# TiagoMSSantos/MobileRayTracer

Hardware: AMD Instinct MI355X
Metric: Mrays/s + ms/frame, Conference OBJ 1920×1080 4spp, 1/2/4/8 GPU (higher is better)
Workload: dtype f32; 1 GPU; conference_1920x1080_4spp_pathtracer_depth5; rendered_pixels=2058240, spp=4, max_depth=5, samples_light=1, parallelism=single GPU

## Files before the change

### include/mobilert_amd.h

```cpp
#ifndef MOBILERT_AMD_H
#define MOBILERT_AMD_H

#include <stddef.h>
#include <stdint.h>

#ifdef __cplusplus
extern "C" {
#endif

typedef struct mrt_renderer mrt_renderer;

typedef struct mrt_config {
    int32_t width;
    int32_t height;
    int32_t threads;
    int32_t shader;
    int32_t sceneIndex;
    int32_t samplesPixel;
    int32_t samplesLight;
    int32_t repeats;
    int32_t accelerator;
    int32_t printStdOut;
    const char *objFilePath;
    const char *mtlFilePath;
// ... 138 lines not shown
int mrt_set_pixel_sampler(mrt_renderer *r, int32_t kind, float value);
int mrt_set_max_point(mrt_renderer *r, const float *maxPoint);
typedef struct mrt_view {
    int32_t kind;
    float position[3], lookAt[3], up[3];
    float a, b;
} mrt_view;
int mrt_render_views(mrt_renderer *r, const mrt_view *views, int32_t nViews, int32_t *bitmaps);
int mrt_render_views_device(mrt_renderer *r, const mrt_view *views, int32_t nViews,
                            int32_t *d_bitmaps, int32_t *d_packed, void *stream);
int mrt_set_tuning(mrt_renderer *r, int32_t key, int32_t value);
int mrt_get_tuning(const mrt_renderer *r, int32_t key, int32_t *value);
int mrt_primary_hits(mrt_renderer *r, int32_t *kind, int32_t *index, float *t);
int64_t mrt_triangle_bvh(const mrt_config *cfg, float *boxes, int32_t *offsets, int32_t *counts, int32_t *order);
int64_t mrt_walk_tree(const mrt_config *cfg, uint32_t *nodes, float *grid, int32_t *root);
int mrt_walk_stack(const mrt_config *cfg, int32_t *out);
int64_t mrt_plan_spill(int64_t threads, int32_t stackNeed, int64_t availBytes);
int64_t mrt_regular_grid(const mrt_config *cfg, int32_t kind, float *world, int32_t *start, int32_t *items);
int mrt_grid_box_test(int32_t kind, const float *prim, const float *box);
int64_t mrt_decode_texture(const char *path, int32_t *dims, uint8_t *texels);
int mrt_plan_queues(const mrt_queue_plan_request *request, mrt_queue_plan *plan);

int mrt_sample_tables(float *shader, float *sampler, float *trig);

int mrt_kat_slab(const float *boxes, const float *orig, const float *dir, int32_t n, int32_t *out);
int mrt_kat_triangle(const float *tris, const float *orig, const float *dir, int32_t n, int32_t *hit, float *t);
int mrt_kat_accumulate(const float *rgb, int32_t nSlots, int32_t spp, int32_t sampleBase, int32_t width,
                       int32_t height, int32_t mode, int32_t *bitmap, int32_t *launched);
int mrt_trace_rays(mrt_renderer *r, const float *orig, const float *dir, const float *dist, const int32_t *src,
                   int32_t n, int32_t any, int32_t *kind, int32_t *index, float *t);
// ... 142 lines not shown
```

### mobileraytracer_amd/__init__.py

```python
import contextlib
import ctypes
import dataclasses
import threading
import time
from typing import List, Optional

import numpy as np

from . import _native

SHADER_WHITTED = 1
SHADER_PATH_TRACER = 2
ACC_BVH = 3
RAY_DEPTH_MAX = 6


@dataclasses.dataclass
class Config:
    width: int = 256
    height: int = 256
    threads: int = 1
    shader: int = SHADER_WHITTED
    sceneIndex: int = 0
    samplesPixel: int = 1
# ... 662 lines not shown


def walk_tree(config: Config):
    lib = _native.lib()
    c = config.to_c()
    n = lib.mrt_walk_tree(ctypes.byref(c), None, None, None)
    if n < 0:
        raise RuntimeError(lib.mrt_last_error().decode())
    grid = np.empty(6, np.float32)
    root = np.empty(3, np.int32)
    lib.mrt_walk_tree(ctypes.byref(c), None, _ptr(grid), _ptr(root))
    nodes = np.empty((n, 4 * int(root[2])), np.uint32)
    if lib.mrt_walk_tree(ctypes.byref(c), _ptr(nodes), _ptr(grid), _ptr(root)) != n:
        raise RuntimeError(lib.mrt_last_error().decode())
    return nodes, grid, root


def walk_stack(config: Config) -> dict:
    out = np.zeros(6, np.int32)
    c = config.to_c()
    _native.check(_native.lib().mrt_walk_stack(ctypes.byref(c), _ptr(out)))
    return {"need": int(out[0]), "quantized": bool(out[1]), "refDepth": int(out[2]), "walkDepth": int(out[3]),
            "wideDepth": int(out[4]), "spillDepth": int(out[5])}


def plan_spill(threads: int, stack_need: int, avail_bytes: int = 0) -> int:
    n = _native.lib().mrt_plan_spill(int(threads), int(stack_need), int(avail_bytes))
    if n < 0:
        raise RuntimeError(_native.lib().mrt_last_error().decode())
    return int(n)
# ... 280 lines not shown
```

### mobileraytracer_amd/_native.py

```python
import ctypes
import os

_HERE = os.path.dirname(os.path.abspath(__file__))
LIB_PATH = os.environ.get("MOBILERT_LIB") or os.path.join(_HERE, "libmobilert_amd.so")

EXPORTED_SYMBOLS = (
    "mrt_last_error", "mrt_build_stamp", "mrt_create", "mrt_destroy", "mrt_render_frame", "mrt_render_frame_device",
    "mrt_unpack_gathered", "mrt_stop_render", "mrt_get_sample", "mrt_get_total_casted_rays",
    "mrt_get_scene_info", "mrt_set_profiling", "mrt_get_frame_stats", "mrt_primary_hits", "mrt_set_tuning",
    "mrt_get_tuning", "mrt_triangle_bvh", "mrt_walk_tree", "mrt_decode_texture", "mrt_kat_slab", "mrt_kat_triangle",
    "mrt_trace_rays", "mrt_sample_tables", "mrt_regular_grid", "mrt_grid_box_test", "mrt_create_from_memory",
    "mrt_preview_arrays", "mrt_wave_log", "mrt_set_camera", "mrt_set_pixel_sampler", "mrt_set_max_point",
    "mrt_android_read_file", "mrt_android_initialize", "mrt_android_render_into_bitmap",
    "mrt_android_render_into_bitmap_cb", "mrt_android_wait_render", "mrt_android_start_render",
    "mrt_android_stop_render", "mrt_android_finish_render", "mrt_android_state", "mrt_android_fps",
    "mrt_android_time_renderer", "mrt_android_sample", "mrt_android_number_of_lights", "mrt_android_resize",
    "mrt_android_vertices", "mrt_android_colors", "mrt_android_camera", "mrt_android_reset",
    "mrt_get_queue_info", "mrt_plan_queues", "mrt_render_views", "mrt_render_views_device",
    "mrt_kat_accumulate", "mrt_cast_rays_device", "mrt_walk_stack", "mrt_plan_spill",
    "mrt_path_key", "mrt_shade_rays_device", "mrt_camera_rays_device",
    "mrt_cast_hits_device", "mrt_cast_multi_hits_device", "mrt_scene_triangles", "mrt_scene_planes", "mrt_scene_spheres", "mrt_scene_materials",
    "mrt_scene_lights", "mrt_nearest_points_device", "mrt_point_distance", "mrt_kat_point_distance",
    "mrt_neighbours_device", "mrt_overlap_boxes_device", "mrt_box_overlap", "mrt_kat_box_overlap",
    "mrt_sweep_spheres_device", "mrt_sphere_sweep", "mrt_kat_sphere_sweep",
    "mrt_overlap_triangles_device", "mrt_triangle_overlap", "mrt_kat_triangle_overlap",
# ... 192 lines not shown
        "mrt_unpack_gathered": (ctypes.c_int, [vp, vp, vp, vp]),
        "mrt_stop_render": (ctypes.c_int, [vp]),
        "mrt_get_sample": (ctypes.c_int32, [vp]),
        "mrt_get_total_casted_rays": (ctypes.c_uint64, [vp]),
        "mrt_get_scene_info": (ctypes.c_int, [vp, P(MrtSceneInfo)]),
        "mrt_set_profiling": (ctypes.c_int, [vp, ctypes.c_int32]),
        "mrt_get_frame_stats": (ctypes.c_int, [vp, P(MrtFrameStats)]),
        "mrt_get_queue_info": (ctypes.c_int, [vp, vp, ctypes.c_size_t]),
        "mrt_plan_queues": (ctypes.c_int, [P(MrtQueuePlanRequest), P(MrtQueuePlan)]),
        "mrt_wave_log": (ctypes.c_int64, [vp, vp]),
        "mrt_primary_hits": (ctypes.c_int, [vp, vp, vp, vp]),
        "mrt_set_tuning": (ctypes.c_int, [vp, ctypes.c_int32, ctypes.c_int32]),
        "mrt_get_tuning": (ctypes.c_int, [vp, ctypes.c_int32, ctypes.POINTER(ctypes.c_int32)]),
        "mrt_triangle_bvh": (ctypes.c_int64, [vp, vp, vp, vp, vp]),
        "mrt_walk_tree": (ctypes.c_int64, [vp, vp, vp, vp]),
        "mrt_walk_stack": (ctypes.c_int, [vp, vp]),
        "mrt_plan_spill": (ctypes.c_int64, [ctypes.c_int64, ctypes.c_int32, ctypes.c_int64]),
        "mrt_decode_texture": (ctypes.c_int64, [ctypes.c_char_p, vp, vp]),
        "mrt_regular_grid": (ctypes.c_int64, [vp, ctypes.c_int32, vp, vp, vp]),
        "mrt_grid_box_test": (ctypes.c_int, [ctypes.c_int32, vp, vp]),
        "mrt_create_from_memory": (ctypes.c_int, [P(MrtConfig), ctypes.c_char_p, ctypes.c_int64, ctypes.c_char_p,
                                                  ctypes.c_int64, ctypes.c_char_p, ctypes.c_int64, vp, ctypes.c_int32,
                                                  P(vp)]),
        "mrt_preview_arrays": (ctypes.c_int64, [vp, vp, vp, vp]),
        "mrt_set_camera": (ctypes.c_int, [vp, ctypes.c_int32, vp, vp, vp, ctypes.c_float, ctypes.c_float]),
        "mrt_set_pixel_sampler": (ctypes.c_int, [vp, ctypes.c_int32, ctypes.c_float]),
        "mrt_set_max_point": (ctypes.c_int, [vp, vp]),
        "mrt_android_read_file": (None, [ctypes.c_char_p, ctypes.c_char_p, ctypes.c_int64]),
        "mrt_android_initialize": (ctypes.c_int32, [P(MrtAndroidConfig)]),
        "mrt_android_render_into_bitmap": (None, [vp, ctypes.c_int32]),
# ... 59 lines not shown


def lib():
    global _LIB
    if _LIB is None:
        _LIB = load_library()
    return _LIB


def source_stamp():
    import hashlib
    d = os.path.join(_HERE, "csrc")
    srcs = ["mrt_scene.cpp", "mrt_grid.cpp", "mrt_texture.cpp", "mrt_android.cpp", "mrt_queue_plan.cpp", "mrt_kernels.hip",
            "mrt_renderer.hip",
            "mrt_common.hpp", "mrt_device.hpp", "mrt_kernels.hpp", "mrt_trace_ww.hpp", "mrt_trace_packet.hpp",
            "mrt_multi_hit.hpp", "mrt_nearest.hpp", "mrt_neighbours.hpp", "mrt_overlap.hpp", "mrt_sweep.hpp", "mrt_triangle_overlap.hpp", "mrt_scene.hpp", "mrt_queue_plan.hpp", "../../include/mobilert_amd.h", "../../include/mobilert_amd.hpp",
            "../../include/mobilert_android.h"]
    h = hashlib.sha256()
    for f in srcs:
        with open(os.path.join(d, f), "rb") as fh:
            h.update(fh.read())
    return h.hexdigest()[:16]


def build_is_current(library=None):
    return (library or lib()).mrt_build_stamp().decode() == source_stamp()


def check(rc):
    if rc != 0:
        raise RuntimeError(lib().mrt_last_error().decode(errors="replace"))
# ... 1 lines not shown
```

### mobileraytracer_amd/csrc/mrt_device.hpp

```cpp
#pragma once

#include "mrt_common.hpp"

namespace mrt {

constexpr int kBlock = 256;
constexpr int kLdsStackMin = 8;
static_assert((kLdsStackMin & (kLdsStackMin - 1)) == 0, "the LDS stack rings are indexed by a power-of-two mask");

struct DScene {
    const float4* triGeom;
    const float4* triShade;
    const float4* triHead;
    const GNode* triNodes;
    const QNode4* triQNodes;
    const float* triQNodesF;
    const float4* leafBoxes;
    const float4* planes;
    const GNode* planeNodes;
    const float4* spheres;
    const GNode* sphereNodes;
    const float4* lights;
    const float4* mats;
    const float4* tables;
    const float4* vertexDraws;
    const float2* jitterDraws;
    GRoot triRoot, triRootRef, planeRoot, sphereRoot;
    QGrid qgrid;
    int32_t qEnabled;
    int32_t nLights;
    int32_t nMats;
// ... 422 lines not shown
```

### mobileraytracer_amd/csrc/mrt_kernels.hip

```cpp
#include "mrt_kernels.hpp"
#include "mrt_trace_ww.hpp"
#include "mrt_trace_packet.hpp"
#include "mrt_multi_hit.hpp"
#include "mrt_nearest.hpp"
#include "mrt_neighbours.hpp"
#include "mrt_overlap.hpp"
#include "mrt_sweep.hpp"
#include "mrt_triangle_overlap.hpp"

#include <algorithm>
#include <atomic>
#include <utility>

namespace mrt {

__device__ __forceinline__ int laneId() { return static_cast<int>(threadIdx.x & 63u); }

__device__ __forceinline__ int waveExclusiveScan(int v, int* total) {
    const int lane = laneId();
    int x = v;
#pragma unroll
    for (int off = 1; off < 64; off <<= 1) {
        const int y = __shfl_up(x, off, 64);
        if (lane >= off) x += y;
// ... 1844 lines not shown

#define MRT_LAUNCH_WALK(KERNEL, SLOT)                                                                           \
    do {                                                                                                       \
        if (s.variant == 0 || referenceOrderOnly(s)) MRT_LAUNCH_ONE(KERNEL, 0, kCullNone, SLOT);               \
        else if (s.cull == kCullFast) MRT_LAUNCH_ONE(KERNEL, 1, kCullFast, SLOT + 1);                          \
        else if (s.cull == kCullCertified) MRT_LAUNCH_ONE(KERNEL, 1, kCullCertified, SLOT + 2);                \
        else if (s.cull == kCullExact) MRT_LAUNCH_ONE(KERNEL, 1, kCullExact, SLOT + 4);                        \
        else MRT_LAUNCH_ONE(KERNEL, 1, kCullNone, SLOT + 3);                                                   \
    } while (0)

bool packetLevel1(const DScene& s) {
    return s.accel == kAccBVH && s.packet != 0 && s.variant == 1 && (s.cull == kCullNone || s.cull == kCullExact) &&
           !referenceOrderOnly(s);
}

void launchTrace(const DScene& s, const Level& lv, int* counters, int level, int2* gstack, int gdepth,
                 unsigned long long* stats, bool countStats, int maxThreads, hipStream_t st, const RaygenArgs* gen) {
    if (s.accel != kAccBVH) {
        hipLaunchKernelGGL((k_trace_other<false>), dim3(1024), dim3(256), 0, st, s, lv, counters, level);
        return;
    }
    const int gridPct = 100;
    if (level == 1 && packetLevel1(s)) {
        const bool views = gen != nullptr && gen->cams != nullptr;
        const int g = std::max(1, views           ? persistentGrid(k_trace_packet<false, kCullExact, 2>, 16, maxThreads)
                                  : gen != nullptr ? persistentGrid(k_trace_packet<false, kCullExact, 1>, 11, maxThreads)
                                                   : persistentGrid(k_trace_packet<false, kCullExact, 0>, 10, maxThreads));
        const RaygenArgs ra = gen != nullptr ? *gen : RaygenArgs{};
#define MRT_LAUNCH_PACKET(CNT, C, GEN)                                                                        \
        hipLaunchKernelGGL((k_trace_packet<CNT, C, GEN>), dim3(g), dim3(kWalkThreads), 0, st, s, lv, counters, level, \
// ... 260 lines not shown
```

### mobileraytracer_amd/csrc/mrt_kernels.hpp

```cpp
#pragma once

#include "mrt_device.hpp"

namespace mrt {

constexpr int kShaderWhitted = 1;
constexpr int kShaderPathTracer = 2;
constexpr int kShaderDepthMap = 3;
constexpr int kShaderDiffuse = 4;
constexpr int kShaderNoShadows = 5;
constexpr int kMaxLevels = 16;
constexpr int kTraceVariants = 2;
constexpr int kDefaultTraceVariant = 1;
constexpr int kAccNaive = 1;
constexpr int kAccGrid = 2;
constexpr int kAccBVH = 3;
constexpr int kTopNodesMax = 64 * 4 / kWalkWidth;

#ifndef MRT_QUEUE_SEGS
#define MRT_QUEUE_SEGS 8
#endif
constexpr int kQueueSegs = MRT_QUEUE_SEGS;
constexpr int kCntSegStride = 64;
constexpr int kCntPairs = 0;
// ... 132 lines not shown

struct AccumArgs {
    PixelMap map;
    int width;
    int slotBase;
    int nSlots;
    int spp;
    int sampleBase;
    int viewSlots;
    int viewPixels;
};


void launchRaygen(const RaygenArgs& a, const Level& lv, int* counters, hipStream_t st);
bool packetLevel1(const DScene& s);
void launchTrace(const DScene& s, const Level& lv, int* counters, int level, int2* gstack, int gdepth,
                 unsigned long long* stats, bool countStats, int maxThreads, hipStream_t st,
                 const RaygenArgs* gen = nullptr);
void launchShadow(const DScene& s, const Level& lv, int* counters, int level, int2* gstack, int gdepth,
                  unsigned long long* stats, bool countStats, int maxThreads, hipStream_t st, int gridPct = 100);
bool canFuseLevel1(int shader, const DScene& s, const ShadeArgs& a);
void launchTraceShadeFused(int shader, const DScene& s, const Level& lv, const Level& nx, int* counters, int level,
                           const ShadeArgs& a, int2* gstack, int gdepth, int maxThreads, hipStream_t st, bool deadNext,
                           const RaygenArgs& ra);
void launchShade(int shader, const DScene& s, const Level& lv, const Level& nx, int* counters, int level,
                 const ShadeArgs& a, int grid, hipStream_t st, bool deadNext = false,
                 const RaygenArgs* regen = nullptr);
void launchResolve(int shader, const DScene& s, const Level& lv, const Level& nx, int* counters, int level,
                   const ShadeArgs& a, int grid, hipStream_t st, bool deadChildren = false,
                   const TexLevel* texLevels = nullptr);
// ... 144 lines not shown
```

### mobileraytracer_amd/csrc/mrt_renderer.hip

```cpp
#include <algorithm>
#include <atomic>
#include <chrono>
#include <cmath>
#include <condition_variable>
#include <functional>
#include <cstdio>
#include <cstdlib>
#include <cstring>
#include <deque>
#include <exception>
#include <future>
#include <memory>
#include <mutex>
#include <stdexcept>
#include <map>
#include <sstream>
#include <string>
#include <thread>
#include <unordered_map>
#include <vector>

#include "mobilert_amd.h"
#include "mobilert_amd.hpp"
#include "mrt_kernels.hpp"
#include "mrt_nearest.hpp"
#include "mrt_overlap.hpp"
#include "mrt_sweep.hpp"
#include "mrt_triangle_overlap.hpp"
#include "mrt_queue_plan.hpp"
#include "mrt_scene.hpp"

namespace {

#define MRT_HIP(x)                                                                              \
    do {                                                                                        \
        const hipError_t e_ = (x);                                                              \
        if (e_ != hipSuccess) throw std::runtime_error(std::string(#x) + ": " + hipGetErrorString(e_)); \
    } while (0)
// ... 338 lines not shown
    bool queryReady = false;
    int64_t planSlots = 0;
    int planSpp = 0;
    struct ShadeBatch {
        mrt::QueryRays rays;
        const uint32_t* keys;
        float* rgb;
        long long rgbStride;
        int64_t n;
    };
    const ShadeBatch* shade = nullptr;
    hipStream_t stream = nullptr;
    int overlap = 1;
    int skipLast = 1;
    int shadowGridPct = 0;
    int fuseL1Mode = -1;
    int genL1 = 2;
    int resolveAcc = 1;
    int shadeWaitsShadow = 0;
    int refill = 0;
    int64_t shadeLaunches = 0;
    bool walkSkipped = false;
    bool fusedL1 = false;
    int lastShadowRender = 1;
    int walkGridCap = 0;
    unsigned long long* hostStats = nullptr;
    bool countersClean = false, statsClean = false;

    bool keepHost = false;
    std::vector<mrt::HTriangle> hostTris;
// ... 129 lines not shown
    if (d.qEnabled == 0 || qn.empty()) qn.resize(1);
    d.triQNodes = r->sceneMem.upload(qn, st);
    {
        static_assert(kWalkWidth == 4, "packet nodes: 4 children");
        std::vector<float> qf(32 * qn.size(), 0.0F);
        for (size_t k = 0; k < qn.size(); ++k) {
            const QNode4& q = qn[k];
            for (int c = 0; c < kWalkWidth; ++c) {
                const uint32_t w0 = q.q[3 * c], w1 = q.q[3 * c + 1], w2 = q.q[3 * c + 2];
                const uint32_t v[6] = {w0 & 0xFFFFu, w1 & 0xFFFFu, w2 & 0xFFFFu, w0 >> 16, w1 >> 16, w2 >> 16};
                for (int j = 0; j < 6; ++j) qf[32 * k + 6 * static_cast<size_t>(c) + static_cast<size_t>(j)] = static_cast<float>(v[j]);
                std::memcpy(&qf[32 * k + 24 + static_cast<size_t>(c)], &q.ref[c], sizeof(int32_t));
            }
        }
        d.triQNodesF = r->sceneMem.upload(qf, st);
    }
    r->stackNeed = walkStackNeed(r->maxBvhDepth, wideDepth(d.qEnabled != 0, d.triRoot, qn));
    {
        std::string err;
        if (planSpillBytes(r->traceThreads, spillDepth(r->stackNeed), 0, &err) < 0) throw std::runtime_error(err);
    }
    toDeviceBVH(tn, sc.triangles.size(), &g, &d.triRootRef, 0, nullptr, &conesRef);
    {
        std::vector<float4> lb(std::max<size_t>(1, 3 * sc.triangles.size()), make_float4(0.0F, 0.0F, 0.0F, 0.0F));
        for (const HBVHNode& n : tn) {
            if (n.numPrimitives <= 0) continue;
            const size_t f = static_cast<size_t>(n.indexOffset);
            float c[6];
            leafCullRecord(sc.triangles, f, f + static_cast<size_t>(n.numPrimitives), n.box, c);
            lb[3 * f] = make_float4(n.box.mn.x, n.box.mn.y, n.box.mn.z, n.box.mx.x);
// ... 340 lines not shown
        hipEvent_t e;
        MRT_HIP(hipEventCreateWithFlags(&e, hipEventDisableTiming));
        p.syncPool.push_back(e);
    }
    return p.syncPool[i];
}

hipEvent_t poolEvent(mrt_renderer::Pipe& p) {
    const size_t i = p.evCount++;
    while (p.evPool.size() <= i) {
        hipEvent_t e;
        MRT_HIP(hipEventCreate(&e));
        p.evPool.push_back(e);
    }
    return p.evPool[i];
}

void renderPass(mrt_renderer* r, int32_t* dBitmap, int32_t* dPacked, hipStream_t st, int sampleBase, int spp) {
    using namespace mrt;
    const mrt_renderer::ShadeBatch* batch = r->shade;
    const int shader = r->shader;
    const bool timing = (r->profileFlags & 1) != 0;
    const bool counting = (r->profileFlags & 2) != 0;
    mrt_renderer::Pipe& pp = r->pipe;
    const int spl = std::max(1, r->cfg.samplesLight);
    ShadeArgs sa{r->maxDepth, spl, {r->maxPoint.x, r->maxPoint.y, r->maxPoint.z}, counting ? pp.stats : nullptr};
    const int nLevels = r->nLevels;
    const mrt::PixelMap& map = r->mapByRank[static_cast<size_t>(r->rankIndex)];
    if (!r->statsClean || counting)
        MRT_HIP(hipMemsetAsync(pp.stats, 0, sizeof(unsigned long long) * (kNumStats + (counting ? kWaveLogEntries : 0)), st));
// ... 24 lines not shown
        ra.slotBase = slot0;
        ra.nPaths = nChunk * spp;
        ra.spp = spp;
        ra.sppTotal = r->cfg.samplesPixel;
        setPixelSampler(r, &ra);
        ra.sampleBase = sampleBase;
        if (r->batchCams != nullptr) {
            ra.cams = r->batchCams;
            ra.viewSlots = r->nSlots;
        }
        const double pathsPerLane = static_cast<double>(ra.nPaths) / std::max(1, r->traceThreads);
        r->ds.fuseShade = batch != nullptr ? 0 : r->fuseL1Mode >= 0 ? r->fuseL1Mode : (pathsPerLane < 12.0 ? 1 : 0);
        const bool fuseL1 = batch == nullptr && nLevels >= 1 && !(skipLast && nLevels == 1) &&
                            !(skipLastShade && nLevels == 1) && canFuseLevel1(shader, r->ds, sa);
        r->fusedL1 = fuseL1;
        const bool genL1 = batch == nullptr && !fuseL1 && r->genL1 != 0 && nLevels >= 1 &&
                           !(skipLast && nLevels == 1) && packetLevel1(r->ds);
        const bool regenL1 = genL1 && r->genL1 == 2 && (shader == kShaderWhitted || shader == kShaderPathTracer) &&
                             !(skipLastShade && nLevels == 1);
        ra.storeRays = regenL1 ? 0 : 1;
        if (batch != nullptr) {
            QueryRays q = batch->rays;
            q.base = slot64;
            launchShadeLoad(pp.levels[1], q, r->queryTables, nChunk, batch->keys, pp.counters, st);
        } else if (!fuseL1 && !genL1) {
            launchRaygen(ra, pp.levels[1], pp.counters, st);
        }
        const int walkThreads = r->walkGridCap > 0 ? std::min(r->traceThreads, r->walkGridCap * kBlock)
                                                   : r->traceThreads;
        const int shadowPct = r->shadowGridPct > 0 ? r->shadowGridPct
                              : sb == st            ? 100
                              : pathsPerLane < 4.0  ? 50
                              : pathsPerLane < 8.0  ? 75
                                                    : 70;
        const int shadePerCU = r->shadeGridPerCU >= 0 ? r->shadeGridPerCU : 14;
        r->ds.refill = r->refill > 0 ? r->refill : pathsPerLane < 4.0 ? 48 : 32;
        size_t sync = 0;
        hipEvent_t shadowDone[kMaxLevels + 1] = {};
        const bool lastOnRender = r->lastShadowRender != 0 && sb != st && nLevels >= 2;
        for (int l = 1; l <= nLevels; ++l) {
            if (timing) MRT_HIP(hipEventRecord(poolEvent(pp), st));
            const bool fused = fuseL1 && l == 1;
            if (fused) {
                launchTraceShadeFused(shader, r->ds, pp.levels[l], pp.levels[l + 1], pp.counters, l, sa, pp.gstack,
                                      r->gdepth, walkThreads, st, skipLastShade && l + 1 == nLevels, ra);
                ++r->shadeLaunches;
            }
            if (!fused && !(skipLast && l == nLevels))
                launchTrace(r->ds, pp.levels[l], pp.counters, l, pp.gstack, r->gdepth, pp.stats, counting,
                            walkThreads, st, genL1 && l == 1 ? &ra : nullptr);
            if (timing) MRT_HIP(hipEventRecord(poolEvent(pp), st));
            if (r->shadeWaitsShadow != 0 && sb != st && l >= 3) MRT_HIP(hipStreamWaitEvent(st, shadowDone[l - 2], 0));
            const bool onRender = lastOnRender && l + 1 >= nLevels;
            const hipStream_t ss = onRender ? st : sb;
            if (!fused && !(skipLastShade && l == nLevels)) {
                launchShade(shader, r->ds, pp.levels[l], pp.levels[l + 1], pp.counters, l, sa,
                            shadePerCU > 0 ? r->cus * shadePerCU : r->workGrid, st,
                            skipLastShade && l + 1 == nLevels, regenL1 && l == 1 ? &ra : nullptr);
                ++r->shadeLaunches;
            }
            if (timing) MRT_HIP(hipEventRecord(poolEvent(pp), st));
            if (sb != st && !onRender) {
                const hipEvent_t shaded = syncEvent(pp, sync++);
                MRT_HIP(hipEventRecord(shaded, st));
// ... 1508 lines not shown
        r->ds.tailDonate = value;
        return 0;
    }
    if (key == 16 && (value == 0 || value == 1)) {
        if (value == 1 && r->stackNeed > mrt::kPacketStack) {
            gLastError = "packet walk: the walk tree needs a deeper stack";
            return -1;
        }
        r->ds.packet = value;
        return 0;
    }
    if (key == 17 && value >= -1 && value <= 1) {
        r->fuseL1Mode = value;
        return 0;
    }
    if (key == 27 && (value == 0 || value == 1)) {
        r->lastShadowRender = value;
        return 0;
    }
    if (key == 33 && value >= 0 && value <= 2) {
        r->genL1 = value;
        return 0;
    }
    if (key == 34 && (value == 0 || value == 1)) {
        r->resolveAcc = value;
        return 0;
    }
    if (key == 35 && (value == 0 || value == 1)) {
        r->shadeWaitsShadow = value;
        return 0;
// ... 177 lines not shown
                                                 : walkTreeOver(tn);
        if (!toQuantizedBVH4(wn, sc.triangles.size(), &r, kTopNodesMax, &top, &g, &qn, nullptr,
                             cost.empty() ? nullptr : &cost))
            throw std::runtime_error("walk tree not quantizable (non-finite boxes)");
        n = static_cast<int64_t>(qn.size());
        if (nodes != nullptr) std::memcpy(nodes, qn.data(), qn.size() * sizeof(QNode4));
        if (grid != nullptr) {
            std::memcpy(grid, g.origin, sizeof(g.origin));
            std::memcpy(grid + 3, g.step, sizeof(g.step));
        }
        if (root != nullptr) {
            root[0] = r.ref;
            root[1] = r.count;
            root[2] = kWalkWidth;
        }
    });
    return rc == 0 ? n : -1;
}

int mrt_walk_stack(const mrt_config* cfg, int32_t* out) {
    using namespace mrt;
    return guarded([&] {
        HScene sc;
        const float ratio = cfg->height > 0 ? static_cast<float>(cfg->width) / static_cast<float>(cfg->height) : 1.0F;
        GCamera cam{};
        if (cfg->sceneIndex >= 0 && cfg->sceneIndex <= 3) {
            sc = builtinScene(cfg->sceneIndex);
            cam = builtinCamera(cfg->sceneIndex, ratio);
        } else {
            std::string err;
// ... 121 lines not shown
        case 8: *value = r->ds.tailDonate; return 0;
        case 9: *value = r->refill; return 0;
        case 10: *value = r->ds.leanShade; return 0;
        case 11: *value = r->shadeGridPerCU; return 0;
        case 16: *value = r->ds.packet; return 0;
        case 17: *value = r->fuseL1Mode; return 0;
        case 27: *value = r->lastShadowRender; return 0;
        case 33: *value = r->genL1; return 0;
        case 34: *value = r->resolveAcc; return 0;
        case 35: *value = r->shadeWaitsShadow; return 0;
        case 28: *value = r->walkGridCap; return 0;
        case 37: *value = r->queueBudgetMiB; return 0;
        case 38: *value = r->queueGrowthPct; return 0;
        case 39: *value = r->queueSlack; return 0;
        case 40: *value = r->stackNeed; return 0;
        default: break;
    }
    gLastError = "unknown tuning key";
    return -1;
}

int mrt_get_frame_stats(const mrt_renderer* r, mrt_frame_stats* s) {
    *s = r->last;
    return 0;
}

int mrt_get_queue_info(const mrt_renderer* r, mrt_queue_info* out, size_t size) {
    using namespace mrt;
    if (r == nullptr || out == nullptr) {
        gLastError = "mrt_get_queue_info: null argument";
// ... 78 lines not shown
                r->countersClean = false;
                RaygenArgs ra{};
                ra.cam = r->cam;
                ra.map = r->mapByRank[static_cast<size_t>(r->rankIndex)];
                ra.tables = r->ds.tables;
                ra.jitter = r->ds.jitterDraws;
                ra.width = r->cfg.width;
                ra.height = r->cfg.height;
                ra.slotBase = slot0;
                ra.nPaths = n;
                ra.spp = 1;
                ra.sppTotal = r->cfg.samplesPixel;
                setPixelSampler(r, &ra);
                ra.sampleBase = 0;
                launchRaygen(ra, pp.levels[1], pp.counters, st);
                launchTrace(r->ds, pp.levels[1], pp.counters, 1, pp.gstack, r->gdepth, pp.stats, false, r->traceThreads, st);
                launchDumpHits(pp.levels[1], n, dk, di, dt, st);
                MRT_HIP(hipMemcpyAsync(hk.data(), dk, sizeof(int32_t) * n, hipMemcpyDeviceToHost, st));
                MRT_HIP(hipMemcpyAsync(hi.data(), di, sizeof(int32_t) * n, hipMemcpyDeviceToHost, st));
                MRT_HIP(hipMemcpyAsync(ht.data(), dt, sizeof(float) * n, hipMemcpyDeviceToHost, st));
                MRT_HIP(hipStreamSynchronize(st));
                for (int q = 0; q < n; ++q) {
                    int x, y;
                    slotToXYHost(units, prefix, slot0 + q, &x, &y);
                    const size_t pix = static_cast<size_t>(y) * static_cast<size_t>(r->cfg.width) + static_cast<size_t>(x);
                    int32_t k = hk[static_cast<size_t>(q)], idx = hi[static_cast<size_t>(q)];
                    if (k == kTriangle) idx = r->triOrder[static_cast<size_t>(idx)];
                    if (k == kPlane) idx = r->planeOrder[static_cast<size_t>(idx)];
                    if (k == kSphere) idx = r->sphereOrder[static_cast<size_t>(idx)];
                    kind[pix] = k;
                    index[pix] = idx;
// ... 404 lines not shown
```

### mobileraytracer_amd/csrc/mrt_trace_packet.hpp

```cpp
#pragma once

#include <type_traits>

#include "mrt_trace_ww.hpp"

namespace mrt {

typedef __attribute__((address_space(4))) const uint32_t ConstU32;
__device__ __forceinline__ int4 sload4i(ConstU32* p) {
    return make_int4(static_cast<int>(p[0]), static_cast<int>(p[1]), static_cast<int>(p[2]), static_cast<int>(p[3]));
}
__device__ __forceinline__ float4 sload4f(ConstU32* p) {
    return make_float4(__uint_as_float(p[0]), __uint_as_float(p[1]), __uint_as_float(p[2]), __uint_as_float(p[3]));
}

__device__ __forceinline__ void pinSgprs(float4 v) { asm volatile("" ::"s"(v.x), "s"(v.y), "s"(v.z), "s"(v.w)); }
__device__ __forceinline__ void pinSgprs(int4 v) { asm volatile("" ::"s"(v.x), "s"(v.y), "s"(v.z), "s"(v.w)); }

struct PacketTri {
    float4 a, ab, ac;
    __device__ __forceinline__ void pin() const {
        asm volatile("" ::"s"(a.x), "s"(a.y), "s"(a.z), "s"(ab.x), "s"(ab.y), "s"(ab.z));
        asm volatile("" ::"s"(ac.x), "s"(ac.y), "s"(ac.z));
    }
// ... 64 lines not shown
};
#endif
struct OnePacket {
    int done = 0;
    __device__ __forceinline__ int next() { return done++ == 0 ? 0 : 64; }
};
template <bool kCount, int kCull, class Stack, class Post = NoPost, class Rays = NoRays, class Fetch = PacketFetch>
__device__ __forceinline__ void tracePacketF(const DScene& s, const float4* __restrict__ rOs,
                                             const float4* __restrict__ rDs, float4* out, int count, Fetch fetch,
                                             Stack& st, TravCount* cnt, int* waveStack, Post post = Post(),
                                             Rays rays = Rays()) {
    static_assert(kCull == kCullNone || kCull == kCullExact, "packet walk: cull modes 0 and 3");
    ConstU32* const qnf = (ConstU32*)(s.triQNodesF);
    ConstU32* const tg = (ConstU32*)(s.triGeom);
    ConstU32* const lb = (ConstU32*)(s.leafBoxes);
    const int lane = static_cast<int>(threadIdx.x & 63u);
    while (true) {
        const int base = uniformInt(fetch.next());
        if (base >= count) break;
        const int i = base + lane;
        const bool valid = i < count;
        v3 o{0, 0, 0}, d{1, 1, 1};
        uint32_t src = 0;
        float4 o4 = make_float4(0.0F, 0.0F, 0.0F, 0.0F), d4 = o4;
        if (valid) {
            if constexpr (std::is_same<Rays, NoRays>::value) {
                o4 = rOs[i];
                d4 = rDs[i];
            } else {
                rays(i, &o4, &d4);
// ... 10 lines not shown
            traverse<kSphere, false>(s, s.sphereNodes, s.sphereRoot, o, d, inv, src, &b, st, cnt);
        }
        float bt = b.t;
        uint32_t bcode = b.code;
        const v3 qa{s.qgrid.step[0] * inv.x, s.qgrid.step[1] * inv.y, s.qgrid.step[2] * inv.z};
        const v3 qb{(s.qgrid.origin[0] - o.x) * inv.x, (s.qgrid.origin[1] - o.y) * inv.y,
                    (s.qgrid.origin[2] - o.z) * inv.z};
        const GRoot& r = s.triRoot;
        float te;
        const bool walking =
            packed && r.count > 0 && slab(r.bmin[0], r.bmin[1], r.bmin[2], r.bmax[0], r.bmax[1], r.bmax[2], o, inv, &te);
        const uint64_t walkers = __ballot(walking);
        int ref = walkers != 0 ? r.ref : kRefDone;
        int sp = 0;
        const int lead = walkers != 0 ? __ffsll(static_cast<unsigned long long>(walkers)) - 1 : 0;
        while (ref != kRefDone) {
            if (ref >= 0) {
                if (kCount && lane == 0) ++cnt->innerIters;
                float4 nf[8];
#pragma unroll
                for (int j = 0; j < 8; ++j) nf[j] = sload4f(qnf + 32 * ref + 4 * j);
#pragma unroll
                for (int j = 0; j < 8; ++j) pinSgprs(nf[j]);
                const auto fw = [&](int k) -> float {
                    const float4 v = nf[k >> 2];
                    const int c = k & 3;
                    return c == 0 ? v.x : c == 1 ? v.y : c == 2 ? v.z : v.w;
                };
                uint32_t key[kWalkWidth];
                int rf[kWalkWidth];
                int n = 0;
// ... 132 lines not shown
```

Measured before the change: 5400 Mrays/s.

## Precompute per-camera screen-space child footprints for coherent primary-ray packet traversal

Adds a per-camera table, built by a new kernel, that projects each quantized BVH child box into the camera's image plane as conservative ordered-integer rectangles, with children sorted by distance. In level-1 packet traversal, when every walking lane shares the camera origin and the wave's ray directions span a small image-space rectangle, inner nodes are tested with four scalar integer rectangle-overlap checks instead of per-lane slab tests. This is meant to cut inner-node ALU and vector work for primary rays. The cost is an extra table build whenever the camera changes, added scene memory, and some risk of conservativeness or precision errors in the rounding and clipping logic.

```diff
diff --git a/include/mobilert_amd.h b/include/mobilert_amd.h
--- a/include/mobilert_amd.h
+++ b/include/mobilert_amd.h
@@ -176,6 +176,8 @@
 int mrt_primary_hits(mrt_renderer *r, int32_t *kind, int32_t *index, float *t);
 int64_t mrt_triangle_bvh(const mrt_config *cfg, float *boxes, int32_t *offsets, int32_t *counts, int32_t *order);
 int64_t mrt_walk_tree(const mrt_config *cfg, uint32_t *nodes, float *grid, int32_t *root);
+int64_t mrt_walk_footprints(const mrt_config *cfg, const mrt_view *view, const uint32_t *nodes, int64_t count,
+                            const float *grid, int32_t *records, double *frame);
 int mrt_walk_stack(const mrt_config *cfg, int32_t *out);
 int64_t mrt_plan_spill(int64_t threads, int32_t stackNeed, int64_t availBytes);
 int64_t mrt_regular_grid(const mrt_config *cfg, int32_t kind, float *world, int32_t *start, int32_t *items);
diff --git a/mobileraytracer_amd/__init__.py b/mobileraytracer_amd/__init__.py
--- a/mobileraytracer_amd/__init__.py
+++ b/mobileraytracer_amd/__init__.py
@@ -700,6 +700,20 @@
     if lib.mrt_walk_tree(ctypes.byref(c), _ptr(nodes), _ptr(grid), _ptr(root)) != n:
         raise RuntimeError(lib.mrt_last_error().decode())
     return nodes, grid, root
+
+
+def walk_footprints(config: Config, nodes: np.ndarray, grid: np.ndarray, camera=None):
+    lib = _native.lib()
+    c = config.to_c()
+    nodes = np.ascontiguousarray(nodes, np.uint32)
+    grid = np.ascontiguousarray(grid, np.float32)
+    n, w = nodes.shape[0], nodes.shape[1] // 4
+    records = np.empty((n, 5 * w), np.int32)
+    frame = np.empty(12, np.float64)
+    view = Renderer._views([camera]) if camera is not None else None
+    if lib.mrt_walk_footprints(ctypes.byref(c), view, _ptr(nodes), n, _ptr(grid), _ptr(records), _ptr(frame)) != n:
+        raise RuntimeError(lib.mrt_last_error().decode())
+    return records, frame
 
 
 def walk_stack(config: Config) -> dict:
diff --git a/mobileraytracer_amd/_native.py b/mobileraytracer_amd/_native.py
--- a/mobileraytracer_amd/_native.py
+++ b/mobileraytracer_amd/_native.py
@@ -8,7 +8,7 @@
     "mrt_last_error", "mrt_build_stamp", "mrt_create", "mrt_destroy", "mrt_render_frame", "mrt_render_frame_device",
     "mrt_unpack_gathered", "mrt_stop_render", "mrt_get_sample", "mrt_get_total_casted_rays",
     "mrt_get_scene_info", "mrt_set_profiling", "mrt_get_frame_stats", "mrt_primary_hits", "mrt_set_tuning",
-    "mrt_get_tuning", "mrt_triangle_bvh", "mrt_walk_tree", "mrt_decode_texture", "mrt_kat_slab", "mrt_kat_triangle",
+    "mrt_get_tuning", "mrt_triangle_bvh", "mrt_walk_tree", "mrt_walk_footprints", "mrt_decode_texture", "mrt_kat_slab", "mrt_kat_triangle",
     "mrt_trace_rays", "mrt_sample_tables", "mrt_regular_grid", "mrt_grid_box_test", "mrt_create_from_memory",
     "mrt_preview_arrays", "mrt_wave_log", "mrt_set_camera", "mrt_set_pixel_sampler", "mrt_set_max_point",
     "mrt_android_read_file", "mrt_android_initialize", "mrt_android_render_into_bitmap",
@@ -231,6 +231,7 @@
         "mrt_get_tuning": (ctypes.c_int, [vp, ctypes.c_int32, ctypes.POINTER(ctypes.c_int32)]),
         "mrt_triangle_bvh": (ctypes.c_int64, [vp, vp, vp, vp, vp]),
         "mrt_walk_tree": (ctypes.c_int64, [vp, vp, vp, vp]),
+        "mrt_walk_footprints": (ctypes.c_int64, [vp, P(MrtView), vp, ctypes.c_int64, vp, vp, vp]),
         "mrt_walk_stack": (ctypes.c_int, [vp, vp]),
         "mrt_plan_spill": (ctypes.c_int64, [ctypes.c_int64, ctypes.c_int32, ctypes.c_int64]),
         "mrt_decode_texture": (ctypes.c_int64, [ctypes.c_char_p, vp, vp]),
@@ -320,7 +321,7 @@
     srcs = ["mrt_scene.cpp", "mrt_grid.cpp", "mrt_texture.cpp", "mrt_android.cpp", "mrt_queue_plan.cpp", "mrt_kernels.hip",
             "mrt_renderer.hip",
             "mrt_common.hpp", "mrt_device.hpp", "mrt_kernels.hpp", "mrt_trace_ww.hpp", "mrt_trace_packet.hpp",
-            "mrt_multi_hit.hpp", "mrt_nearest.hpp", "mrt_neighbours.hpp", "mrt_overlap.hpp", "mrt_sweep.hpp", "mrt_triangle_overlap.hpp", "mrt_scene.hpp", "mrt_queue_plan.hpp", "../../include/mobilert_amd.h", "../../include/mobilert_amd.hpp",
+            "mrt_footprint.hpp", "mrt_multi_hit.hpp", "mrt_nearest.hpp", "mrt_neighbours.hpp", "mrt_overlap.hpp", "mrt_sweep.hpp", "mrt_triangle_overlap.hpp", "mrt_scene.hpp", "mrt_queue_plan.hpp", "../../include/mobilert_amd.h", "../../include/mobilert_amd.hpp",
             "../../include/mobilert_android.h"]
     h = hashlib.sha256()
     for f in srcs:
diff --git a/mobileraytracer_amd/csrc/mrt_device.hpp b/mobileraytracer_amd/csrc/mrt_device.hpp
--- a/mobileraytracer_amd/csrc/mrt_device.hpp
+++ b/mobileraytracer_amd/csrc/mrt_device.hpp
@@ -15,6 +15,10 @@
     const GNode* triNodes;
     const QNode4* triQNodes;
     const float* triQNodesF;
+    const uint32_t* footNodes;
+    float footP[3], footD[3], footR[3], footU[3];
+    float footMaxA, footMaxB;
+    int32_t foot;
     const float4* leafBoxes;
     const float4* planes;
     const GNode* planeNodes;
diff --git a/mobileraytracer_amd/csrc/mrt_footprint.hpp b/mobileraytracer_amd/csrc/mrt_footprint.hpp
--- /dev/null
+++ b/mobileraytracer_amd/csrc/mrt_footprint.hpp
@@ -0,0 +1,170 @@
+#pragma once
+
+#include <cmath>
+
+#include "mrt_common.hpp"
+
+namespace mrt {
+
+constexpr double kFootInflate = 0x1p-19;
+constexpr double kFootAbs = 0x1p-100;
+constexpr double kFootFront = 0x1p-10;
+constexpr float kFootLaneFront = 0.25F;
+constexpr float kFootMargin = 0x1p-17F;
+constexpr int kFootWords = 5 * kWalkWidth;
+constexpr int32_t kFootAll0 = static_cast<int32_t>(0x80000000u), kFootAll1 = 0x7FFFFFFF;
+
+struct FootCam {
+    double p[3], d[3], r[3], u[3];
+};
+
+MRT_HD int32_t footOrdered(float f) {
+    const float z = f + 0.0F;
+#if defined(__HIP_DEVICE_COMPILE__)
+    const int32_t i = __float_as_int(z);
+#else
+    int32_t i;
+    __builtin_memcpy(&i, &z, sizeof(i));
+#endif
+    return i ^ ((i >> 31) & 0x7FFFFFFF);
+}
+MRT_HD float footDown(double x) {
+    float f = static_cast<float>(x);
+    if (static_cast<double>(f) > x) f = nextafterf(f, -INFINITY);
+    return f;
+}
+MRT_HD float footUp(double x) {
+    float f = static_cast<float>(x);
+    if (static_cast<double>(f) < x) f = nextafterf(f, INFINITY);
+    return f;
+}
+
+MRT_HD double footChild(const FootCam& c, const double mn[3], const double mx[3], int32_t out[4]) {
+    double lo[3], hi[3], dist2 = 0.0;
+    for (int k = 0; k < 3; ++k) {
+        const double far = fmax(fabs(mn[k] - c.p[k]), fabs(mx[k] - c.p[k]));
+        const double grow = kFootInflate * far + kFootAbs;
+        lo[k] = (mn[k] - c.p[k]) - grow;
+        hi[k] = (mx[k] - c.p[k]) + grow;
+        const double gap = fmax(fmax(mn[k] - c.p[k], c.p[k] - mx[k]), 0.0);
+        dist2 += gap * gap;
+    }
+    double big = 0.0, near1 = 0.0;
+    for (int k = 0; k < 3; ++k) {
+        big += fmax(fabs(lo[k]), fabs(hi[k]));
+        near1 += fmax(fmax(lo[k], -hi[k]), 0.0);
+    }
+    const double clip = kFootFront * big;
+    bool all = !(near1 > 4.5 * clip);
+    double a0 = INFINITY, a1 = -INFINITY, b0 = INFINITY, b1 = -INFINITY;
+    int vertices = 0;
+    const auto vertex = [&](const double* v) {
+        const double den = (v[0] * c.d[0] + v[1] * c.d[1]) + v[2] * c.d[2];
+        const double a = ((v[0] * c.r[0] + v[1] * c.r[1]) + v[2] * c.r[2]) / den;
+        const double b = ((v[0] * c.u[0] + v[1] * c.u[1]) + v[2] * c.u[2]) / den;
+        const double m = static_cast<double>(kFootMargin) * ((1.0 + fabs(a)) + fabs(b));
+        a0 = fmin(a0, a - m);
+        a1 = fmax(a1, a + m);
+        b0 = fmin(b0, b - m);
+        b1 = fmax(b1, b + m);
+        if (!(den > 0.0)) all = true;
+        ++vertices;
+    };
+    double cv[8][3], den[8];
+    for (int corner = 0; corner < 8; ++corner) {
+        for (int k = 0; k < 3; ++k) cv[corner][k] = ((corner >> k) & 1) ? hi[k] : lo[k];
+        den[corner] = (cv[corner][0] * c.d[0] + cv[corner][1] * c.d[1]) + cv[corner][2] * c.d[2];
+        if (!(den[corner] == den[corner])) all = true;
+        if (den[corner] > clip) vertex(cv[corner]);
+    }
+    for (int corner = 0; corner < 8; ++corner)
+        for (int k = 0; k < 3; ++k) {
+            const int other = corner | (1 << k);
+            if (other == corner || (den[corner] > clip) == (den[other] > clip)) continue;
+            const int f = den[corner] > clip ? corner : other, n = den[corner] > clip ? other : corner;
+            const double s = (den[f] - clip) / (den[f] - den[n]);
+            double x[3];
+            for (int j = 0; j < 3; ++j) x[j] = cv[f][j] + s * (cv[n][j] - cv[f][j]);
+            vertex(x);
+        }
+    if (!all && vertices == 0) {
+        out[0] = out[2] = kFootAll1;
+        out[1] = out[3] = kFootAll0;
+        return dist2;
+    }
+    const float f[4] = {footDown(a0), footUp(a1), footDown(b0), footUp(b1)};
+    for (int k = 0; k < 4; ++k)
+        if (!(fabsf(f[k]) <= 3.0e38F)) all = true;
+    for (int k = 0; k < 4; ++k) out[k] = all ? ((k & 1) ? kFootAll1 : kFootAll0) : footOrdered(f[k]);
+    return dist2;
+}
+
+MRT_HD void footNode(const FootCam& c, const QGrid& g, const QNode4& q, uint32_t* rec) {
+    int32_t ref[kWalkWidth], rect[kWalkWidth][4];
+    double key[kWalkWidth];
+    for (int ch = 0; ch < kWalkWidth; ++ch) {
+        ref[ch] = q.ref[ch];
+        if (ref[ch] == kEmptyChild) {
+            key[ch] = INFINITY;
+            for (int k = 0; k < 4; ++k) rect[ch][k] = (k & 1) ? kFootAll0 : kFootAll1;
+            continue;
+        }
+        double mn[3], mx[3];
+        for (int k = 0; k < 3; ++k) {
+            const uint32_t w = q.q[3 * ch + k];
+            mn[k] = static_cast<double>(g.origin[k]) + static_cast<double>(w & 0xFFFFu) * static_cast<double>(g.step[k]);
+            mx[k] = static_cast<double>(g.origin[k]) + static_cast<double>(w >> 16) * static_cast<double>(g.step[k]);
+        }
+        key[ch] = footChild(c, mn, mx, rect[ch]);
+    }
+    int order[kWalkWidth];
+    for (int ch = 0; ch < kWalkWidth; ++ch) {
+        int at = ch;
+        while (at > 0 && key[order[at - 1]] > key[ch]) {
+            order[at] = order[at - 1];
+            --at;
+        }
+        order[at] = ch;
+    }
+    for (int s = 0; s < kWalkWidth; ++s) {
+        rec[s] = static_cast<uint32_t>(ref[order[s]]);
+        for (int k = 0; k < 4; ++k) rec[kWalkWidth + 4 * s + k] = static_cast<uint32_t>(rect[order[s]][k]);
+    }
+}
+
+inline bool footCamOf(const GCamera& cam, FootCam* out) {
+    if (cam.kind != 0) return false;
+    const double m[3][3] = {{cam.direction.x, cam.direction.y, cam.direction.z},
+                            {cam.right.x, cam.right.y, cam.right.z},
+                            {cam.up.x, cam.up.y, cam.up.z}};
+    double len[3];
+    for (int i = 0; i < 3; ++i) len[i] = std::sqrt(m[i][0] * m[i][0] + m[i][1] * m[i][1] + m[i][2] * m[i][2]);
+    if (!(std::fabs(len[0] - 1.0) <= 1.0e-3 && len[1] >= 0.3 && len[1] <= 4.0 && len[2] >= 0.3 && len[2] <= 4.0)) return false;
+    for (int i = 0; i < 3; ++i)
+        for (int j = i + 1; j < 3; ++j) {
+            const double dotij = m[i][0] * m[j][0] + m[i][1] * m[j][1] + m[i][2] * m[j][2];
+            if (!(std::fabs(dotij) <= 1.0e-3 * len[i] * len[j])) return false;
+        }
+    const auto crossd = [](const double* a, const double* b, double* o) {
+        o[0] = a[1] * b[2] - a[2] * b[1];
+        o[1] = a[2] * b[0] - a[0] * b[2];
+        o[2] = a[0] * b[1] - a[1] * b[0];
+    };
+    double c0[3], c1[3], c2[3];
+    crossd(m[1], m[2], c0);
+    crossd(m[2], m[0], c1);
+    crossd(m[0], m[1], c2);
+    const double det = m[0][0] * c0[0] + m[0][1] * c0[1] + m[0][2] * c0[2];
+    if (!(std::fabs(det) > 0.05)) return false;
+    for (int k = 0; k < 3; ++k) {
+        out->d[k] = c0[k] / det;
+        out->r[k] = c1[k] / det;
+        out->u[k] = c2[k] / det;
+    }
+    out->p[0] = cam.position.x;
+    out->p[1] = cam.position.y;
+    out->p[2] = cam.position.z;
+    return std::isfinite(out->p[0]) && std::isfinite(out->p[1]) && std::isfinite(out->p[2]);
+}
+
+}
diff --git a/mobileraytracer_amd/csrc/mrt_kernels.hip b/mobileraytracer_amd/csrc/mrt_kernels.hip
--- a/mobileraytracer_amd/csrc/mrt_kernels.hip
+++ b/mobileraytracer_amd/csrc/mrt_kernels.hip
@@ -1882,6 +1882,21 @@
            !referenceOrderOnly(s);
 }
 
+__global__ __launch_bounds__(256) void k_footprints(const QNode4* nodes, QGrid grid, int nNodes, FootCam c, uint32_t* table) {
+    const int i = static_cast<int>(blockIdx.x * blockDim.x + threadIdx.x);
+    if (i >= nNodes) return;
+    uint32_t rec[kFootWords];
+    footNode(c, grid, nodes[i], rec);
+    uint4* out = reinterpret_cast<uint4*>(table + static_cast<size_t>(kFootWords) * static_cast<size_t>(i));
+#pragma unroll
+    for (int k = 0; k < kFootWords / 4; ++k) out[k] = make_uint4(rec[4 * k], rec[4 * k + 1], rec[4 * k + 2], rec[4 * k + 3]);
+}
+
+void launchFootprints(const DScene& s, int nNodes, const FootCam& c, uint32_t* table, hipStream_t st) {
+    if (nNodes <= 0) return;
+    hipLaunchKernelGGL(k_footprints, dim3((nNodes + 255) / 256), dim3(256), 0, st, s.triQNodes, s.qgrid, nNodes, c, table);
+}
+
 void launchTrace(const DScene& s, const Level& lv, int* counters, int level, int2* gstack, int gdepth,
                  unsigned long long* stats, bool countStats, int maxThreads, hipStream_t st, const RaygenArgs* gen) {
     if (s.accel != kAccBVH) {
diff --git a/mobileraytracer_amd/csrc/mrt_kernels.hpp b/mobileraytracer_amd/csrc/mrt_kernels.hpp
--- a/mobileraytracer_amd/csrc/mrt_kernels.hpp
+++ b/mobileraytracer_amd/csrc/mrt_kernels.hpp
@@ -170,6 +170,8 @@
 
 void launchRaygen(const RaygenArgs& a, const Level& lv, int* counters, hipStream_t st);
 bool packetLevel1(const DScene& s);
+struct FootCam;
+void launchFootprints(const DScene& s, int nNodes, const FootCam& c, uint32_t* table, hipStream_t st);
 void launchTrace(const DScene& s, const Level& lv, int* counters, int level, int2* gstack, int gdepth,
                  unsigned long long* stats, bool countStats, int maxThreads, hipStream_t st,
                  const RaygenArgs* gen = nullptr);
diff --git a/mobileraytracer_amd/csrc/mrt_renderer.hip b/mobileraytracer_amd/csrc/mrt_renderer.hip
--- a/mobileraytracer_amd/csrc/mrt_renderer.hip
+++ b/mobileraytracer_amd/csrc/mrt_renderer.hip
@@ -22,6 +22,7 @@
 
 #include "mobilert_amd.h"
 #include "mobilert_amd.hpp"
+#include "mrt_footprint.hpp"
 #include "mrt_kernels.hpp"
 #include "mrt_nearest.hpp"
 #include "mrt_overlap.hpp"
@@ -390,6 +391,13 @@
     int overlap = 1;
     int skipLast = 1;
     int shadowGridPct = 0;
+    int footMode = 1;
+    uint32_t* footTable = nullptr;
+    int footNodeCount = 0;
+    bool footMade = false;
+    mrt::GCamera footCamera{};
+    hipStream_t footStream = nullptr;
+    int64_t footBuilds = 0;
     int fuseL1Mode = -1;
     int genL1 = 2;
     int resolveAcc = 1;
@@ -549,6 +557,11 @@
             }
         }
         d.triQNodesF = r->sceneMem.upload(qf, st);
+        r->footNodeCount = d.qEnabled != 0 ? static_cast<int>(qn.size()) : 0;
+        r->footTable = r->sceneMem.alloc<uint32_t>(static_cast<size_t>(kFootWords) * qn.size());
+        r->footMade = false;
+        d.footNodes = r->footTable;
+        d.foot = 0;
     }
     r->stackNeed = walkStackNeed(r->maxBvhDepth, wideDepth(d.qEnabled != 0, d.triRoot, qn));
     {
@@ -919,6 +932,33 @@
         p.evPool.push_back(e);
     }
     return p.evPool[i];
+}
+
+mrt::DScene level1Scene(mrt_renderer* r, bool frame, hipStream_t st) {
+    using namespace mrt;
+    DScene d = r->ds;
+    d.foot = 0;
+    FootCam fc;
+    if (!frame || r->footMode == 0 || r->views != 1 || r->batchCams != nullptr || r->footNodeCount <= 0 ||
+        !packetLevel1(d) || !footCamOf(r->cam, &fc))
+        return d;
+    if (!r->footMade || st != r->footStream || std::memcmp(&r->cam, &r->footCamera, sizeof(GCamera)) != 0) {
+        launchFootprints(d, r->footNodeCount, fc, r->footTable, st);
+        r->footCamera = r->cam;
+        r->footStream = st;
+        r->footMade = true;
+        ++r->footBuilds;
+    }
+    for (int k = 0; k < 3; ++k) {
+        d.footP[k] = static_cast<float>(fc.p[k]);
+        d.footD[k] = static_cast<float>(fc.d[k]);
+        d.footR[k] = static_cast<float>(fc.r[k]);
+        d.footU[k] = static_cast<float>(fc.u[k]);
+    }
+    d.footMaxA = 24.0F * std::fabs(r->cam.hFov) / static_cast<float>(std::max(1, r->cfg.width));
+    d.footMaxB = 24.0F * std::fabs(r->cam.vFov) / static_cast<float>(std::max(1, r->cfg.height));
+    d.foot = 1;
+    return d;
 }
 
 void renderPass(mrt_renderer* r, int32_t* dBitmap, int32_t* dPacked, hipStream_t st, int sampleBase, int spp) {
@@ -973,6 +1013,7 @@
         const bool fuseL1 = batch == nullptr && nLevels >= 1 && !(skipLast && nLevels == 1) &&
                             !(skipLastShade && nLevels == 1) && canFuseLevel1(shader, r->ds, sa);
         r->fusedL1 = fuseL1;
+        const DScene dsL1 = level1Scene(r, batch == nullptr, st);
         const bool genL1 = batch == nullptr && !fuseL1 && r->genL1 != 0 && nLevels >= 1 &&
                            !(skipLast && nLevels == 1) && packetLevel1(r->ds);
         const bool regenL1 = genL1 && r->genL1 == 2 && (shader == kShaderWhitted || shader == kShaderPathTracer) &&
@@ -1001,12 +1042,12 @@
             if (timing) MRT_HIP(hipEventRecord(poolEvent(pp), st));
             const bool fused = fuseL1 && l == 1;
             if (fused) {
-                launchTraceShadeFused(shader, r->ds, pp.levels[l], pp.levels[l + 1], pp.counters, l, sa, pp.gstack,
+                launchTraceShadeFused(shader, dsL1, pp.levels[l], pp.levels[l + 1], pp.counters, l, sa, pp.gstack,
                                       r->gdepth, walkThreads, st, skipLastShade && l + 1 == nLevels, ra);
                 ++r->shadeLaunches;
             }
             if (!fused && !(skipLast && l == nLevels))
-                launchTrace(r->ds, pp.levels[l], pp.counters, l, pp.gstack, r->gdepth, pp.stats, counting,
+                launchTrace(l == 1 ? dsL1 : r->ds, pp.levels[l], pp.counters, l, pp.gstack, r->gdepth, pp.stats, counting,
                             walkThreads, st, genL1 && l == 1 ? &ra : nullptr);
             if (timing) MRT_HIP(hipEventRecord(poolEvent(pp), st));
             if (r->shadeWaitsShadow != 0 && sb != st && l >= 3) MRT_HIP(hipStreamWaitEvent(st, shadowDone[l - 2], 0));
@@ -2545,6 +2586,10 @@
         r->fuseL1Mode = value;
         return 0;
     }
+    if (key == 41 && (value == 0 || value == 1)) {
+        r->footMode = value;
+        return 0;
+    }
     if (key == 27 && (value == 0 || value == 1)) {
         r->lastShadowRender = value;
         return 0;
@@ -2752,6 +2797,46 @@
             root[1] = r.count;
             root[2] = kWalkWidth;
         }
+    });
+    return rc == 0 ? n : -1;
+}
+
+int64_t mrt_walk_footprints(const mrt_config* cfg, const mrt_view* view, const uint32_t* nodes, int64_t count,
+                            const float* grid, int32_t* records, double* frame) {
+    using namespace mrt;
+    int64_t n = -1;
+    const int rc = guarded([&] {
+        if (cfg == nullptr || nodes == nullptr || grid == nullptr || count < 0)
+            throw std::runtime_error("mrt_walk_footprints: null argument");
+        GCamera cam{};
+        if (view != nullptr) {
+            cam = cameraOf("mrt_walk_footprints", view->kind, view->position, view->lookAt, view->up, view->a, view->b);
+        } else {
+            const float ratio = cfg->height > 0 ? static_cast<float>(cfg->width) / static_cast<float>(cfg->height) : 1.0F;
+            std::string err;
+            if (cfg->sceneIndex >= 0 && cfg->sceneIndex <= 3)
+                cam = builtinCamera(cfg->sceneIndex, ratio);
+            else if (!loadCameraFile(cfg->camFilePath ? cfg->camFilePath : "", ratio, &cam, &err))
+                throw std::runtime_error(err);
+        }
+        FootCam fc;
+        if (!footCamOf(cam, &fc)) throw std::runtime_error("mrt_walk_footprints: the camera has no footprints (orthographic, or looking along its up vector)");
+        QGrid g{};
+        std::memcpy(g.origin, grid, sizeof(g.origin));
+        std::memcpy(g.step, grid + 3, sizeof(g.step));
+        if (records != nullptr)
+            for (int64_t i = 0; i < count; ++i) {
+                QNode4 q;
+                std::memcpy(&q, nodes + (sizeof(QNode4) / sizeof(uint32_t)) * static_cast<size_t>(i), sizeof(q));
+                footNode(fc, g, q, reinterpret_cast<uint32_t*>(records) + static_cast<size_t>(kFootWords) * static_cast<size_t>(i));
+            }
+        if (frame != nullptr) {
+            std::memcpy(frame, fc.p, sizeof(fc.p));
+            std::memcpy(frame + 3, fc.d, sizeof(fc.d));
+            std::memcpy(frame + 6, fc.r, sizeof(fc.r));
+            std::memcpy(frame + 9, fc.u, sizeof(fc.u));
+        }
+        n = count;
     });
     return rc == 0 ? n : -1;
 }
@@ -2903,6 +2988,8 @@
         case 38: *value = r->queueGrowthPct; return 0;
         case 39: *value = r->queueSlack; return 0;
         case 40: *value = r->stackNeed; return 0;
+        case 41: *value = r->footMode; return 0;
+        case 42: *value = static_cast<int32_t>(r->footBuilds); return 0;
         default: break;
     }
     gLastError = "unknown tuning key";
@@ -3011,7 +3098,8 @@
                 setPixelSampler(r, &ra);
                 ra.sampleBase = 0;
                 launchRaygen(ra, pp.levels[1], pp.counters, st);
-                launchTrace(r->ds, pp.levels[1], pp.counters, 1, pp.gstack, r->gdepth, pp.stats, false, r->traceThreads, st);
+                launchTrace(level1Scene(r, true, st), pp.levels[1], pp.counters, 1, pp.gstack, r->gdepth, pp.stats, false,
+                            r->traceThreads, st);
                 launchDumpHits(pp.levels[1], n, dk, di, dt, st);
                 MRT_HIP(hipMemcpyAsync(hk.data(), dk, sizeof(int32_t) * n, hipMemcpyDeviceToHost, st));
                 MRT_HIP(hipMemcpyAsync(hi.data(), di, sizeof(int32_t) * n, hipMemcpyDeviceToHost, st));
diff --git a/mobileraytracer_amd/csrc/mrt_trace_packet.hpp b/mobileraytracer_amd/csrc/mrt_trace_packet.hpp
--- a/mobileraytracer_amd/csrc/mrt_trace_packet.hpp
+++ b/mobileraytracer_amd/csrc/mrt_trace_packet.hpp
@@ -2,6 +2,7 @@
 
 #include <type_traits>
 
+#include "mrt_footprint.hpp"
 #include "mrt_trace_ww.hpp"
 
 namespace mrt {
@@ -102,6 +103,7 @@
     ConstU32* const qnf = (ConstU32*)(s.triQNodesF);
     ConstU32* const tg = (ConstU32*)(s.triGeom);
     ConstU32* const lb = (ConstU32*)(s.leafBoxes);
+    ConstU32* const fnodes = (ConstU32*)(s.footNodes);
     const int lane = static_cast<int>(threadIdx.x & 63u);
     while (true) {
         const int base = uniformInt(fetch.next());
@@ -142,7 +144,67 @@
         int ref = walkers != 0 ? r.ref : kRefDone;
         int sp = 0;
         const int lead = walkers != 0 ? __ffsll(static_cast<unsigned long long>(walkers)) - 1 : 0;
+        bool foot = false;
+        int pa0 = 0, pa1 = 0, pb0 = 0, pb1 = 0;
+        if (s.foot != 0 && walkers != 0) {
+            const float den = (d.x * s.footD[0] + d.y * s.footD[1]) + d.z * s.footD[2];
+            const float l1 = (fabsf(d.x) + fabsf(d.y)) + fabsf(d.z);
+            const float a = ((d.x * s.footR[0] + d.y * s.footR[1]) + d.z * s.footR[2]) / den;
+            const float bb = ((d.x * s.footU[0] + d.y * s.footU[1]) + d.z * s.footU[2]) / den;
+            const bool mine = o.x == s.footP[0] && o.y == s.footP[1] && o.z == s.footP[2] && den >= kFootLaneFront * l1 &&
+                              fabsf(a) <= 1.0e30F && fabsf(bb) <= 1.0e30F;
+            if (__ballot(walking && !mine) == 0) {
+                constexpr float kInf = __builtin_inff();
+                float a0 = walking ? a : kInf, a1 = walking ? a : -kInf, b0 = walking ? bb : kInf, b1 = walking ? bb : -kInf;
+                for (int off = 32; off > 0; off >>= 1) {
+                    a0 = fminf(a0, __shfl_xor(a0, off, 64));
+                    a1 = fmaxf(a1, __shfl_xor(a1, off, 64));
+                    b0 = fminf(b0, __shfl_xor(b0, off, 64));
+                    b1 = fmaxf(b1, __shfl_xor(b1, off, 64));
+                }
+                const float m = kFootMargin * ((1.0F + fmaxf(fabsf(a0), fabsf(a1))) + fmaxf(fabsf(b0), fabsf(b1)));
+                pa0 = uniformInt(footOrdered(a0 - m));
+                pa1 = uniformInt(footOrdered(a1 + m));
+                pb0 = uniformInt(footOrdered(b0 - m));
+                pb1 = uniformInt(footOrdered(b1 + m));
+                foot = uniformInt(a1 - a0 <= s.footMaxA && b1 - b0 <= s.footMaxB ? 1 : 0) != 0;
+            }
+        }
         while (ref != kRefDone) {
+            if (ref >= 0 && foot) {
+                if (kCount && lane == 0) ++cnt->innerIters;
+                static_assert(kWalkWidth == 4, "footprint records: 4 children");
+                ConstU32* const rec = fnodes + kFootWords * ref;
+                const int4 rr = sload4i(rec);
+                const int4 c0 = sload4i(rec + 4), c1 = sload4i(rec + 8), c2 = sload4i(rec + 12), c3 = sload4i(rec + 16);
+                pinSgprs(rr);
+                pinSgprs(c0);
+                pinSgprs(c1);
+                pinSgprs(c2);
+                pinSgprs(c3);
+                if (kCount && walking)
+                    cnt->nodes += static_cast<uint32_t>((rr.x != kEmptyChild) + (rr.y != kEmptyChild) + (rr.z != kEmptyChild) +
+                                                        (rr.w != kEmptyChild));
+                const auto over = [&](int4 c) { return (c.x <= pa1) & (c.y >= pa0) & (c.z <= pb1) & (c.w >= pb0); };
+                const bool in0 = over(c0), in1 = over(c1), in2 = over(c2), in3 = over(c3);
+                if (in3 & (in0 | in1 | in2)) {
+                    if (lane == 0) waveStack[sp] = rr.w;
+                    ++sp;
+                }
+                if (in2 & (in0 | in1)) {
+                    if (lane == 0) waveStack[sp] = rr.z;
+                    ++sp;
+                }
+                if (in1 & in0) {
+                    if (lane == 0) waveStack[sp] = rr.y;
+                    ++sp;
+                }
+                if (in0 | in1 | in2 | in3)
+                    ref = in0 ? rr.x : in1 ? rr.y : in2 ? rr.z : rr.w;
+                else
+                    ref = sp > 0 ? uniformInt(waveStack[--sp]) : kRefDone;
+                continue;
+            }
             if (ref >= 0) {
                 if (kCount && lane == 0) ++cnt->innerIters;
                 float4 nf[8];
```

Result: no change. 5379 Mrays/s (-0.4%).
